# JinPLu/VeloxSeg

Measured on AMD Instinct MI355X. Metric: training patches/s on 128^3 2-mod volumes (fwd+loss+bwd+allreduce+AdamW), higher is better.
Workload: dtype f32

## Files before the change

veloxseg_amd/csrc/expand_mfma.hip:

```cpp
#include "vx_common.h"
#include <type_traits>
#include "../../include/veloxseg_hip.h"

__device__ __forceinline__ int vx_xcd_tile(int bid, int nb) { return (nb & 7) == 0 ? (bid & 7) * (nb >> 3) + (bid >> 3) : bid; }

typedef float vx_f4 __attribute__((ext_vector_type(4)));

__global__ void __launch_bounds__(256) vx_weight_tap_major_k(const float* __restrict__ w, float* __restrict__ wt, int Cout, int Cin, int K3) {
    const long n = (long)Cout * Cin * K3;
    const long e = (long)blockIdx.x * 256 + threadIdx.x;
    if (e >= n) return;
    const int ci = (int)(e % Cin);
    const int co = (int)((e / Cin) % Cout);
    const int t = (int)(e / ((long)Cin * Cout));
    wt[e] = w[((long)co * Cin + ci) * K3 + t];
}

__global__ void __launch_bounds__(256) vx_to_channels_last16_k(const float* __restrict__ x, float* __restrict__ xcl, long V) {
    __shared__ float tile[16][65];
    const int b = blockIdx.y;
    const long v0 = (long)blockIdx.x * 64;
    for (int e = threadIdx.x; e < 16 * 64; e += 256) {
        const int c = e / 64, k = e % 64;
        tile[c][k] = (v0 + k < V) ? x[((long)b * 16 + c) * V + v0 + k] : 0.0f;
// ... 603 lines not shown
    const float* __restrict__ xb = x + (long)b * 16 * V;
    for (int e = threadIdx.x; e < 2 * 648; e += 256) {
        const int hv = e % 648, half = e / 648;
        const int hw = hv % 18, hh = (hv / 18) % 6, hd = hv / 108;
        const int qd = d0 - 1 + hd, qh = h0 - 1 + hh, qw = w0 - 1 + hw;
        const bool ok = (unsigned)qd < (unsigned)D && (unsigned)qh < (unsigned)H && (unsigned)qw < (unsigned)W;
        const float* __restrict__ src = xb + (long)(8 * half) * V + (ok ? ((long)qd * H + qh) * W + qw : 0);
        float v[8];
#pragma unroll
        for (int j = 0; j < 8; ++j) v[j] = src[(long)j * V];
        uint4 pk = make_uint4(0u, 0u, 0u, 0u);
        if (ok) pk = make_uint4(vx_pack_bf16(v[0], v[1]), vx_pack_bf16(v[2], v[3]), vx_pack_bf16(v[4], v[5]), vx_pack_bf16(v[6], v[7]));
        xh[e] = pk;
    }
    __syncthreads();
    const long FH = 4L * H, FW = 4L * W;
    const long fplane = (4L * D) * FH * FW;
    for (int g = 0; g < Cc * 4; ++g) {
        const int c = g >> 2, s1 = g & 3;
        const int co_base = g * 16;
        vx_f4 acc[4];
#pragma unroll
        for (int m = 0; m < 4; ++m) acc[m] = (vx_f4){0.f, 0.f, 0.f, 0.f};
        const uint4* __restrict__ wg = wimg + (long)g * 14 * 64 + lane;
#pragma unroll 2
        for (int p = 0; p < 14; ++p) {
            const int t = 2 * p + (q >> 1);
            const int tt = t < 27 ? t : 26;
            const int tw = tt % 3, th = (tt / 3) % 3, td = tt / 9;
            const uint4 av = wg[p * 64];
            const uint4* __restrict__ xt = xh + (q & 1) * 648 + ((wave + td) * 6 + th) * 18 + r + tw;
            uint4 bv[4];
#pragma unroll
            for (int m = 0; m < 4; ++m) bv[m] = xt[m * 18];
#pragma unroll
            for (int m = 0; m < 4; ++m) acc[m] = __builtin_amdgcn_mfma_f32_16x16x32_bf16(vx_as_bf8(av), vx_as_bf8(bv[m]), acc[m], 0, 0, 0);
        }
        const float4 bb = bias ? *reinterpret_cast<const float4*>(bias + co_base + 4 * q) : make_float4(0.f, 0.f, 0.f, 0.f);
        TY* __restrict__ yb = y + ((long)b * Cc + c) * fplane + ((long)(4 * (d0 + wave) + s1) * FH + q) * FW + 4 * (w0 + r);
#pragma unroll
        for (int m = 0; m < 4; ++m)
            if (w0 + r < W) vx_st4(yb, (long)(4 * (h0 + m)) * FW, make_float4(acc[m][0] + bb.x, acc[m][1] + bb.y, acc[m][2] + bb.z, acc[m][3] + bb.w));
    }
}

extern "C" int vx_expand_fwd_mfma_bf16_h(const float* x, const float* w, const float* bias, float* wt_ws, void* y, int B, int Cc, int D, int H, int W, int y_h16, void* stream) {
    VX_REQUIRE(x && w && wt_ws && y && B > 0 && Cc > 0 && D > 0 && H > 0 && W > 0, "vx_expand_fwd_mfma_bf16: bad args");
    if (D % 4 != 0 || H % 4 != 0 || W % 4 != 0) return 1;
    hipStream_t st = (hipStream_t)stream;
    const int groups = Cc * 4;
    vx_expand_wimg_bf16_k<<<vx_cdiv((long)groups * 14 * 64 * 4, 256), 256, 0, st>>>(w, reinterpret_cast<uint32_t*>(wt_ws), groups, 0);
    const long nblk = (long)B * (D / 4) * (H / 4) * ((W + 15) / 16);
    if (y_h16) vx_expand_fwd_bf16_k<vx_bf16><<<dim3((unsigned)nblk), 256, 0, st>>>(x, reinterpret_cast<const uint4*>(wt_ws), bias, (vx_bf16*)y, B, Cc, D, H, W);
    else vx_expand_fwd_bf16_k<float><<<dim3((unsigned)nblk), 256, 0, st>>>(x, reinterpret_cast<const uint4*>(wt_ws), bias, (float*)y, B, Cc, D, H, W);
    VX_LAUNCH_CHECK("vx_expand_fwd_mfma_bf16");
    return 0;
}
extern "C" int vx_expand_fwd_mfma_bf16(const float* x, const float* w, const float* bias, float* wt_ws, float* y, int B, int Cc, int D, int H, int W, void* stream) {
    return vx_expand_fwd_mfma_bf16_h(x, w, bias, wt_ws, y, B, Cc, D, H, W, 0, stream);
}

template <typename TD>
__global__ void __launch_bounds__(256) vx_expand_bwd_data_bf16_k(const TD* __restrict__ dyf, const uint4* __restrict__ wimg, float* __restrict__ dx,
                                                                 int B, int Cc, int D, int H, int W, int accumulate) {
    extern __shared__ __attribute__((aligned(16))) unsigned short vx_halo_h[];
    const int lane = threadIdx.x & 63;
    const int wave = __builtin_amdgcn_readfirstlane((int)(threadIdx.x >> 6));
    const int r = lane & 15, q = lane >> 4;
    const int nTw = (W + 15) / 16, nTh = H / 4, nTd = D / 4;
    int tile = vx_xcd_tile(blockIdx.x, gridDim.x);
    const int tw_i = tile % nTw; tile /= nTw;
    const int th_i = tile % nTh; tile /= nTh;
    const int td_i = tile % nTd;
    const int b = tile / nTd;
    const int d0 = td_i * 4, h0 = th_i * 4, w0 = tw_i * 16;
    const long V = (long)D * H * W;
    const long FH = 4L * H, FW = 4L * W;
    const long fplane = (4L * D) * FH * FW;
    const TD* __restrict__ dyb = dyf + (long)b * Cc * fplane;
    vx_f4 acc[4];
#pragma unroll
    for (int m = 0; m < 4; ++m) acc[m] = (vx_f4){0.f, 0.f, 0.f, 0.f};
    long goff[11];
    int loff[11];
#pragma unroll
    for (int u = 0; u < 11; ++u) {
        const int e = min((int)threadIdx.x + u * 256, 144 * 18 - 1);
        const int f4 = e % 18, row = e / 18;
        const int s2 = row & 3, hh = (row >> 2) % 6, hd = row / 24;
        const int qd = d0 - 1 + hd, qh = h0 - 1 + hh, qw = w0 - 1 + f4;
        const bool ok = (unsigned)qd < (unsigned)D && (unsigned)qh < (unsigned)H && (unsigned)qw < (unsigned)W;
        goff[u] = ok ? ((long)(4 * qd) * FH + 4 * qh + s2) * FW + 4 * qw : -1;
        loff[u] = ((int)threadIdx.x + u * 256 < 144 * 18) ? (e / 18) * 72 + (e % 18) * 4 : -1;
    }
    for (int c = 0; c < Cc; ++c) {
        for (int s1 = 0; s1 < 4; ++s1) {
            __syncthreads();
            {
                uint2 v[11];
#pragma unroll
                for (int u = 0; u < 11; ++u) {
                    const long o = (long)c * fplane + (goff[u] >= 0 ? goff[u] + (long)s1 * FH * FW : 0);
                    if constexpr (std::is_same<TD, vx_bf16>::value) {
                        const uint2 t_ = *reinterpret_cast<const uint2*>(dyb + o);
                        v[u] = goff[u] >= 0 ? t_ : make_uint2(0u, 0u);
                    } else {
                        const float4 t_ = *reinterpret_cast<const float4*>(dyb + o);
                        v[u] = goff[u] >= 0 ? make_uint2(vx_pack_bf16(t_.x, t_.y), vx_pack_bf16(t_.z, t_.w)) : make_uint2(0u, 0u);
                    }
                }
#pragma unroll
                for (int u = 0; u < 11; ++u)
                    if (loff[u] >= 0) *reinterpret_cast<uint2*>(vx_halo_h + loff[u]) = v[u];
            }
            __syncthreads();
            const uint4* __restrict__ wg = wimg + (long)(c * 4 + s1) * 14 * 64 + lane;
#pragma unroll 2
            for (int p = 0; p < 14; ++p) {
                const int t = 2 * p + (q >> 1);
                const int tt = t < 27 ? t : 26;
                const int tw = tt % 3, th = (tt / 3) % 3, td = tt / 9;
                const uint4 bv = wg[p * 64];
                const int hd = wave - td + 2;
                const int s2 = 2 * (q & 1);
                const unsigned short* __restrict__ ht = vx_halo_h + ((hd * 6 + (2 - th)) * 4 + s2) * 72 + (r - tw + 2) * 4;
                uint4 av[4];
#pragma unroll
                for (int m = 0; m < 4; ++m) {
                    const uint2 lo = *reinterpret_cast<const uint2*>(ht + m * 4 * 72);
                    const uint2 hi = *reinterpret_cast<const uint2*>(ht + m * 4 * 72 + 72);
                    av[m] = make_uint4(lo.x, lo.y, hi.x, hi.y);
                }
#pragma unroll
                for (int m = 0; m < 4; ++m) acc[m] = __builtin_amdgcn_mfma_f32_16x16x32_bf16(vx_as_bf8(av[m]), vx_as_bf8(bv), acc[m], 0, 0, 0);
            }
        }
    }
#pragma unroll
    for (int m = 0; m < 4; ++m) {
        const long pbase = ((long)(d0 + wave) * H + (h0 + m)) * W + w0 + 4 * q;
        float* dst = dx + ((long)b * 16 + r) * V + pbase;
        if (w0 + 4 * q >= W) continue;
        float4 o = make_float4(acc[m][0], acc[m][1], acc[m][2], acc[m][3]);
        if (accumulate) { const float4 old = *reinterpret_cast<float4*>(dst); o.x += old.x; o.y += old.y; o.z += old.z; o.w += old.w; }
        *reinterpret_cast<float4*>(dst) = o;
    }
}

extern "C" int vx_expand_bwd_data_mfma_bf16_h(const void* dy_fine, const float* w, float* wt_ws, float* dx, int B, int Cc, int D, int H, int W,
                                              int accumulate, int dy_h16, void* stream) {
    VX_REQUIRE(dy_fine && w && wt_ws && dx && B > 0 && Cc > 0 && D > 0 && H > 0 && W > 0, "vx_expand_bwd_data_mfma_bf16: bad args");
    if (D % 4 != 0 || H % 4 != 0 || W % 4 != 0) return 1;
    hipStream_t st = (hipStream_t)stream;
    const int groups = Cc * 4;
    vx_expand_wimg_bf16_k<<<vx_cdiv((long)groups * 14 * 64 * 4, 256), 256, 0, st>>>(w, reinterpret_cast<uint32_t*>(wt_ws), groups, 1);
    const long nblk = (long)B * (D / 4) * (H / 4) * ((W + 15) / 16);
    if (dy_h16) vx_expand_bwd_data_bf16_k<vx_bf16><<<dim3((unsigned)nblk), 256, 6 * 6 * 4 * 72 * sizeof(unsigned short), st>>>((const vx_bf16*)dy_fine, reinterpret_cast<const uint4*>(wt_ws), dx, B, Cc, D, H, W, accumulate);
    else vx_expand_bwd_data_bf16_k<float><<<dim3((unsigned)nblk), 256, 6 * 6 * 4 * 72 * sizeof(unsigned short), st>>>((const float*)dy_fine, reinterpret_cast<const uint4*>(wt_ws), dx, B, Cc, D, H, W, accumulate);
    VX_LAUNCH_CHECK("vx_expand_bwd_data_mfma_bf16");
    return 0;
}
extern "C" int vx_expand_bwd_data_mfma_bf16(const float* dy_fine, const float* w, float* wt_ws, float* dx, int B, int Cc, int D, int H, int W,
                                            int accumulate, void* stream) {
    return vx_expand_bwd_data_mfma_bf16_h(dy_fine, w, wt_ws, dx, B, Cc, D, H, W, accumulate, 0, stream);
}


template <int NS>
__device__ __forceinline__ void vx_split8(const float (&v)[8], uint4 (&out)[NS]) {
    float r[8];
#pragma unroll
    for (int j = 0; j < 8; ++j) r[j] = v[j];
#pragma unroll
    for (int s = 0; s < NS; ++s) {
        typedef __bf16 bf2 __attribute__((ext_vector_type(2)));
        uint32_t pk[4];
#pragma unroll
        for (int j2 = 0; j2 < 4; ++j2) {
            const bf2 h = {(__bf16)r[2 * j2], (__bf16)r[2 * j2 + 1]};
            pk[j2] = __builtin_bit_cast(uint32_t, h);
            if (s + 1 < NS) { r[2 * j2] -= (float)h[0]; r[2 * j2 + 1] -= (float)h[1]; }
        }
        out[s] = make_uint4(pk[0], pk[1], pk[2], pk[3]);
    }
}
template <int NS>
__global__ void __launch_bounds__(256) vx_expand_wimg_split_k(const float* __restrict__ w, uint32_t* __restrict__ img, int groups, int backward) {
    const long n = (long)groups * 14 * 64 * 4;
    const long e = (long)blockIdx.x * 256 + threadIdx.x;
    if (e >= n) return;
    const int jp = (int)(e & 3), lane = (int)((e >> 2) & 63);
    const long t = e >> 8;
    const int p = (int)(t % 14), g = (int)(t / 14);
    const int r = lane & 15, q = lane >> 4;
    const int tap = 2 * p + (q >> 1);
    float v[2] = {0.f, 0.f};
    if (tap < 27)
        for (int u = 0; u < 2; ++u) {
            const int j = 2 * jp + u;
            int co, ci;
            if (backward) { co = 16 * g + 4 * (2 * (q & 1) + (j >> 2)) + (j & 3); ci = r; }
            else { co = 16 * g + r; ci = 8 * (q & 1) + j; }
            v[u] = w[((long)co * 16 + ci) * 27 + tap];
        }
#pragma unroll
    for (int s = 0; s < NS; ++s) {
        typedef __bf16 bf2 __attribute__((ext_vector_type(2)));
        const bf2 h = {(__bf16)v[0], (__bf16)v[1]};
        img[(long)s * n + e] = __builtin_bit_cast(uint32_t, h);
        v[0] -= (float)h[0]; v[1] -= (float)h[1];
    }
}
typedef _Float16 vx_h8 __attribute__((ext_vector_type(8)));
__device__ __forceinline__ vx_h8 vx_as_h8(uint4 v) { return __builtin_bit_cast(vx_h8, v); }
__device__ __forceinline__ uint32_t vx_pack_h2(float a, float b) {
    typedef _Float16 h2 __attribute__((ext_vector_type(2)));
    const h2 v = {(_Float16)a, (_Float16)b};
    return __builtin_bit_cast(uint32_t, v);
}
__device__ __forceinline__ float vx_h2_lo(uint32_t p) { typedef _Float16 h2 __attribute__((ext_vector_type(2))); return (float)__builtin_bit_cast(h2, p)[0]; }
__device__ __forceinline__ float vx_h2_hi(uint32_t p) { typedef _Float16 h2 __attribute__((ext_vector_type(2))); return (float)__builtin_bit_cast(h2, p)[1]; }
__device__ __forceinline__ int vx_exp16(float m) {
    if (!(m > 0.0f) || !(m < 3.0e38f)) return 0;
    const int e = 14 - ilogbf(m);
    return e > 100 ? 100 : (e < -100 ? -100 : e);
}
__global__ void __launch_bounds__(256) vx_expand_wmax_k(const float* __restrict__ w, long n, float* __restrict__ out) {
    __shared__ float sm[4];
    float mx = 0.0f;
    const long n4 = n >> 2;
    for (long i = (long)blockIdx.x * 256 + threadIdx.x; i < n4; i += (long)gridDim.x * 256) {
        const float4 t = reinterpret_cast<const float4*>(w)[i];
        mx = fmaxf(mx, fmaxf(fmaxf(fabsf(t.x), fabsf(t.y)), fmaxf(fabsf(t.z), fabsf(t.w))));
    }
    if (blockIdx.x == 0)
        for (long i = 4 * n4 + threadIdx.x; i < n; i += 256) mx = fmaxf(mx, fabsf(w[i]));
    mx = vx_wave_max(mx);
    if ((threadIdx.x & 63) == 0) sm[threadIdx.x >> 6] = mx;
    __syncthreads();
    if (threadIdx.x == 0) out[4 + blockIdx.x] = fmaxf(fmaxf(sm[0], sm[1]), fmaxf(sm[2], sm[3]));
}
__device__ __forceinline__ int vx_expand_wexp(const float* __restrict__ ew) { return vx_exp16(__uint_as_float(reinterpret_cast<const unsigned*>(ew)[1])); }
static inline int vx_expand_wmax_launch(const float* w, long n, float* ew, hipStream_t st) {
    int nb = (int)((n / 4 + 255) / 256);
    if (nb > 64) nb = 64;
    if (nb < 1) nb = 1;
    vx_expand_wmax_k<<<nb, 256, 0, st>>>(w, n, ew);
    return nb;
}
__global__ void __launch_bounds__(256) vx_expand_wimg_f16_k(const float* __restrict__ w, uint32_t* __restrict__ img, const float* __restrict__ ew, int groups, int backward,
                                                            int nparts, float* __restrict__ ew_out) {
    const long n = (long)groups * 14 * 64 * 4;
    const long e = (long)blockIdx.x * 256 + threadIdx.x;
    int wexp;
    if (nparts > 0) {
        float mx = 0.0f;
        for (int i = 0; i < nparts; ++i) mx = fmaxf(mx, ew_out[4 + i]);
        wexp = vx_exp16(mx);
        if (e == 0) { reinterpret_cast<unsigned*>(ew_out)[0] = 0u; reinterpret_cast<unsigned*>(ew_out)[1] = __float_as_uint(mx); }
    } else wexp = vx_expand_wexp(ew);
    if (e >= n) return;
    const float sc = ldexpf(1.0f, wexp);
    const int jp = (int)(e & 3), lane = (int)((e >> 2) & 63);
    const long t = e >> 8;
    const int p = (int)(t % 14), g = (int)(t / 14);
    const int r = lane & 15, q = lane >> 4;
    const int tap = 2 * p + (q >> 1);
    float v[2] = {0.f, 0.f};
    if (tap < 27)
        for (int u = 0; u < 2; ++u) {
            const int j = 2 * jp + u;
            int co, ci;
            if (backward) { co = 16 * g + 4 * (2 * (q & 1) + (j >> 2)) + (j & 3); ci = r; }
            else { co = 16 * g + r; ci = 8 * (q & 1) + j; }
            v[u] = w[((long)co * 16 + ci) * 27 + tap] * sc;
        }
    const uint32_t h0 = vx_pack_h2(v[0], v[1]);
    img[e] = h0;
    img[n + e] = vx_pack_h2(v[0] - vx_h2_lo(h0), v[1] - vx_h2_hi(h0));
}
__device__ __forceinline__ void vx_split8_h(const float (&v)[8], float sc, uint4 (&out)[2]) {
    uint32_t p0[4], p1[4];
#pragma unroll
    for (int j2 = 0; j2 < 4; ++j2) {
        const float a = v[2 * j2] * sc, b = v[2 * j2 + 1] * sc;
        p0[j2] = vx_pack_h2(a, b);
        p1[j2] = vx_pack_h2(a - vx_h2_lo(p0[j2]), b - vx_h2_hi(p0[j2]));
    }
    out[0] = make_uint4(p0[0], p0[1], p0[2], p0[3]);
    out[1] = make_uint4(p1[0], p1[1], p1[2], p1[3]);
}
__device__ __forceinline__ float vx_block_max_256(float m, float* __restrict__ scratch) {
    m = vx_wave_max(m);
    if ((threadIdx.x & 63) == 0) scratch[threadIdx.x >> 6] = m;
    __syncthreads();
    return fmaxf(fmaxf(scratch[0], scratch[1]), fmaxf(scratch[2], scratch[3]));
}

template <int NS> struct VxSplitTerms;
template <> struct VxSplitTerms<1> { static constexpr int N = 1; static constexpr int A[1] = {0}; static constexpr int W[1] = {0}; };
template <> struct VxSplitTerms<2> { static constexpr int N = 3; static constexpr int A[3] = {1, 0, 0}; static constexpr int W[3] = {0, 1, 0}; };
template <> struct VxSplitTerms<3> { static constexpr int N = 6; static constexpr int A[6] = {1, 2, 0, 1, 0, 0}; static constexpr int W[6] = {1, 0, 2, 0, 1, 0}; };

template <int NS, bool F16 = false>
__global__ void __launch_bounds__(256) vx_expand_fwd_split_k(const float* __restrict__ x, const uint4* __restrict__ wimg, const float* __restrict__ bias,
                                                             float* __restrict__ y, int B, int Cc, int D, int H, int W, const float* __restrict__ ew = nullptr) {
    extern __shared__ __attribute__((aligned(16))) uint4 vx_xs[];
    using TT = VxSplitTerms<NS>;
    const int lane = threadIdx.x & 63;
    const int wave = __builtin_amdgcn_readfirstlane((int)(threadIdx.x >> 6));
    const int r = lane & 15, q = lane >> 4;
    const int nTw = (W + 15) / 16, nTh = H / 4, nTd = D / 4;
    int tile = vx_xcd_tile(blockIdx.x, gridDim.x);
    const int tw_i = tile % nTw; tile /= nTw;
    const int th_i = tile % nTh; tile /= nTh;
    const int td_i = tile % nTd;
    const int b = tile / nTd;
    const int d0 = td_i * 4, h0 = th_i * 4, w0 = tw_i * 16;
    const long V = (long)D * H * W;
    const float* __restrict__ xb = x + (long)b * 16 * V;
    float fscale = 1.0f;
    if constexpr (F16) {
        float v[6][8];
        float mx = 0.0f;
#pragma unroll
        for (int i = 0; i < 6; ++i) {
            const int e = (int)threadIdx.x + i * 256;
            const int ec = e < 2 * 648 ? e : 0;
            const int hv = ec % 648, half = ec / 648;
            const int hw = hv % 18, hh = (hv / 18) % 6, hd = hv / 108;
            const int qd = d0 - 1 + hd, qh = h0 - 1 + hh, qw = w0 - 1 + hw;
            const bool ok = e < 2 * 648 && (unsigned)qd < (unsigned)D && (unsigned)qh < (unsigned)H && (unsigned)qw < (unsigned)W;
            const float* __restrict__ src = xb + (long)(8 * half) * V + (ok ? ((long)qd * H + qh) * W + qw : 0);
#pragma unroll
            for (int j = 0; j < 8; ++j) { const float t_ = src[(long)j * V]; v[i][j] = ok ? t_ : 0.0f; mx = fmaxf(mx, fabsf(v[i][j])); }
        }
        float* scratch = reinterpret_cast<float*>(vx_xs + NS * (2 * 648));
        const int ex = vx_exp16(vx_block_max_256(mx, scratch));
        const float sc = ldexpf(1.0f, ex);
        fscale = ldexpf(1.0f, -(ex + vx_expand_wexp(ew)));
#pragma unroll
        for (int i = 0; i < 6; ++i) {
            const int e = (int)threadIdx.x + i * 256;
            if (e < 2 * 648) {
                uint4 pk[2];
                vx_split8_h(v[i], sc, pk);
                vx_xs[e] = pk[0];
                vx_xs[2 * 648 + e] = pk[1];
            }
        }
    } else {
    for (int e = threadIdx.x; e < 2 * 648; e += 256) {
        const int hv = e % 648, half = e / 648;
        const int hw = hv % 18, hh = (hv / 18) % 6, hd = hv / 108;
        const int qd = d0 - 1 + hd, qh = h0 - 1 + hh, qw = w0 - 1 + hw;
        const bool ok = (unsigned)qd < (unsigned)D && (unsigned)qh < (unsigned)H && (unsigned)qw < (unsigned)W;
        const float* __restrict__ src = xb + (long)(8 * half) * V + (ok ? ((long)qd * H + qh) * W + qw : 0);
        float v[8];
#pragma unroll
        for (int j = 0; j < 8; ++j) { const float t_ = src[(long)j * V]; v[j] = ok ? t_ : 0.0f; }
        uint4 pk[NS];
        vx_split8<NS>(v, pk);
#pragma unroll
        for (int s = 0; s < NS; ++s) vx_xs[s * (2 * 648) + e] = pk[s];
    }
    }
    __syncthreads();
    const long FH = 4L * H, FW = 4L * W;
    const long fplane = (4L * D) * FH * FW;
    const long wn = (long)Cc * 4 * 14 * 64;
    for (int g = 0; g < Cc * 4; ++g) {
        const int c = g >> 2, s1 = g & 3;
        const int co_base = g * 16;
        vx_f4 acc[4];
#pragma unroll
        for (int m = 0; m < 4; ++m) acc[m] = (vx_f4){0.f, 0.f, 0.f, 0.f};
        const uint4* __restrict__ wg = wimg + (long)g * 14 * 64 + lane;
#pragma unroll 2
        for (int p = 0; p < 14; ++p) {
            const int t = 2 * p + (q >> 1);
            const int tt = t < 27 ? t : 26;
            const int tw = tt % 3, th = (tt / 3) % 3, td = tt / 9;
            uint4 av[NS], bv[NS][4];
#pragma unroll
            for (int s = 0; s < NS; ++s) {
                av[s] = wg[s * wn + p * 64];
                const uint4* __restrict__ xt = vx_xs + s * (2 * 648) + (q & 1) * 648 + ((wave + td) * 6 + th) * 18 + r + tw;
#pragma unroll
                for (int m = 0; m < 4; ++m) bv[s][m] = xt[m * 18];
            }
#pragma unroll
            for (int k = 0; k < TT::N; ++k)
#pragma unroll
                for (int m = 0; m < 4; ++m) {
                    if constexpr (F16) acc[m] = __builtin_amdgcn_mfma_f32_16x16x32_f16(vx_as_h8(av[TT::W[k]]), vx_as_h8(bv[TT::A[k]][m]), acc[m], 0, 0, 0);
                    else acc[m] = __builtin_amdgcn_mfma_f32_16x16x32_bf16(vx_as_bf8(av[TT::W[k]]), vx_as_bf8(bv[TT::A[k]][m]), acc[m], 0, 0, 0);
                }
        }
        if constexpr (F16) {
#pragma unroll
            for (int m = 0; m < 4; ++m) acc[m] *= fscale;
        }
        const float4 bb = bias ? *reinterpret_cast<const float4*>(bias + co_base + 4 * q) : make_float4(0.f, 0.f, 0.f, 0.f);
        float* __restrict__ yb = y + ((long)b * Cc + c) * fplane + ((long)(4 * (d0 + wave) + s1) * FH + q) * FW + 4 * (w0 + r);
#pragma unroll
        for (int m = 0; m < 4; ++m)
            if (w0 + r < W) *reinterpret_cast<float4*>(yb + (long)(4 * (h0 + m)) * FW) = make_float4(acc[m][0] + bb.x, acc[m][1] + bb.y, acc[m][2] + bb.z, acc[m][3] + bb.w);
    }
}

template <int NS>
__device__ __forceinline__ void vx_split4(const float4 v, uint2 (&out)[NS]) {
    float r[4] = {v.x, v.y, v.z, v.w};
#pragma unroll
    for (int s = 0; s < NS; ++s) {
        typedef __bf16 bf2 __attribute__((ext_vector_type(2)));
        const bf2 h0 = {(__bf16)r[0], (__bf16)r[1]}, h1 = {(__bf16)r[2], (__bf16)r[3]};
        out[s] = make_uint2(__builtin_bit_cast(uint32_t, h0), __builtin_bit_cast(uint32_t, h1));
        if (s + 1 < NS) { r[0] -= (float)h0[0]; r[1] -= (float)h0[1]; r[2] -= (float)h1[0]; r[3] -= (float)h1[1]; }
    }
}
template <int NS, bool F16 = false>
__global__ void __launch_bounds__(256) vx_expand_bwd_data_split_k(const float* __restrict__ dyf, const uint4* __restrict__ wimg, float* __restrict__ dx,
                                                                  int B, int Cc, int D, int H, int W, int accumulate, const float* __restrict__ ew = nullptr) {
    extern __shared__ __attribute__((aligned(16))) uint2 vx_hs[];
    using TT = VxSplitTerms<NS>;
    const int lane = threadIdx.x & 63;
    const int wave = __builtin_amdgcn_readfirstlane((int)(threadIdx.x >> 6));
    const int r = lane & 15, q = lane >> 4;
    const int nTw = (W + 15) / 16, nTh = H / 4, nTd = D / 4;
    int tile = vx_xcd_tile(blockIdx.x, gridDim.x);
    const int tw_i = tile % nTw; tile /= nTw;
    const int th_i = tile % nTh; tile /= nTh;
    const int td_i = tile % nTd;
    const int b = tile / nTd;
    const int d0 = td_i * 4, h0 = th_i * 4, w0 = tw_i * 16;
    const long V = (long)D * H * W;
    const long FH = 4L * H, FW = 4L * W;
    const long fplane = (4L * D) * FH * FW;
    const float* __restrict__ dyb = dyf + (long)b * Cc * fplane;
    const long wn = (long)Cc * 4 * 14 * 64;
    vx_f4 acc[4];
    vx_f4 tot[4];
#pragma unroll
    for (int m = 0; m < 4; ++m) { acc[m] = (vx_f4){0.f, 0.f, 0.f, 0.f}; tot[m] = (vx_f4){0.f, 0.f, 0.f, 0.f}; }
    int soff[11];
    unsigned okm = 0;
#pragma unroll
    for (int u = 0; u < 11; ++u) {
        const int e = min((int)threadIdx.x + u * 256, 144 * 18 - 1);
        const int f4 = e % 18, row = e / 18;
        const int s2 = row & 3, hh = (row >> 2) % 6, hd = row / 24;
        const int qd = d0 - 1 + hd, qh = h0 - 1 + hh, qw = w0 - 1 + f4;
        const bool ok = (unsigned)qd < (unsigned)D && (unsigned)qh < (unsigned)H && (unsigned)qw < (unsigned)W;
        soff[u] = ok ? (int)(((long)(4 * qd) * FH + 4 * qh + s2) * FW + 4 * qw) : 0;
        okm |= (ok ? 1u : 0u) << u;
    }
    const long s1stride = FH * FW;
    for (int c = 0; c < Cc; ++c) {
        for (int s1 = 0; s1 < 4; ++s1) {
            __syncthreads();
            float gscale = 1.0f;
            {
                float4 v[11];
                const float* __restrict__ cb_ = dyb + (long)c * fplane + (long)s1 * s1stride;
#pragma unroll
                for (int u = 0; u < 11; ++u) {
                    const bool ok = (okm >> u) & 1u;
                    const float4 t_ = *reinterpret_cast<const float4*>(ok ? cb_ + soff[u] : dyb);
                    v[u] = ok ? t_ : make_float4(0.f, 0.f, 0.f, 0.f);
                }
                if constexpr (F16) {
                    float mx = 0.0f;
#pragma unroll
                    for (int u = 0; u < 11; ++u) mx = fmaxf(mx, fmaxf(fmaxf(fabsf(v[u].x), fabsf(v[u].y)), fmaxf(fabsf(v[u].z), fabsf(v[u].w))));
                    const int ex = vx_exp16(vx_block_max_256(mx, reinterpret_cast<float*>(vx_hs + NS * (144 * 18))));
                    const float sc = ldexpf(1.0f, ex);
                    gscale = ldexpf(1.0f, -(ex + vx_expand_wexp(ew)));
#pragma unroll
                    for (int u = 0; u < 11; ++u) {
                        const int e = (int)threadIdx.x + u * 256;
                        if (e < 144 * 18) {
                            const float a0 = v[u].x * sc, a1 = v[u].y * sc, a2 = v[u].z * sc, a3 = v[u].w * sc;
                            const uint32_t l0 = vx_pack_h2(a0, a1), h0 = vx_pack_h2(a2, a3);
                            vx_hs[e] = make_uint2(l0, h0);
                            vx_hs[144 * 18 + e] = make_uint2(vx_pack_h2(a0 - vx_h2_lo(l0), a1 - vx_h2_hi(l0)), vx_pack_h2(a2 - vx_h2_lo(h0), a3 - vx_h2_hi(h0)));
                        }
                    }
                } else {
#pragma unroll
                for (int u = 0; u < 11; ++u) {
                    const int e = (int)threadIdx.x + u * 256;
                    if (e < 144 * 18) {
                        uint2 pc[NS];
                        vx_split4<NS>(v[u], pc);
#pragma unroll
                        for (int s = 0; s < NS; ++s) vx_hs[s * (144 * 18) + e] = pc[s];
                    }
                }
                }
            }
            __syncthreads();
            const uint4* __restrict__ wg = wimg + (long)(c * 4 + s1) * 14 * 64 + lane;
#pragma unroll 2
            for (int p = 0; p < 14; ++p) {
                const int t = 2 * p + (q >> 1);
                const int tt = t < 27 ? t : 26;
                const int tw = tt % 3, th = (tt / 3) % 3, td = tt / 9;
                uint4 bv[NS];
#pragma unroll
                for (int s = 0; s < NS; ++s) bv[s] = wg[s * wn + p * 64];
                const int hd = wave - td + 2;
                const int s2 = 2 * (q & 1);
                const uint2* __restrict__ ht = vx_hs + ((hd * 6 + (2 - th)) * 4 + s2) * 18 + (r - tw + 2);
                uint4 av[4][NS];
#pragma unroll
                for (int s = 0; s < NS; ++s)
#pragma unroll
                    for (int m = 0; m < 4; ++m) {
                        const uint2 lo = ht[s * (144 * 18) + m * 4 * 18], hi = ht[s * (144 * 18) + m * 4 * 18 + 18];
                        av[m][s] = make_uint4(lo.x, lo.y, hi.x, hi.y);
                    }
#pragma unroll
                for (int k = 0; k < TT::N; ++k)
#pragma unroll
                    for (int m = 0; m < 4; ++m) {
                        if constexpr (F16) acc[m] = __builtin_amdgcn_mfma_f32_16x16x32_f16(vx_as_h8(av[m][TT::A[k]]), vx_as_h8(bv[TT::W[k]]), acc[m], 0, 0, 0);
                        else acc[m] = __builtin_amdgcn_mfma_f32_16x16x32_bf16(vx_as_bf8(av[m][TT::A[k]]), vx_as_bf8(bv[TT::W[k]]), acc[m], 0, 0, 0);
                    }
            }
            if constexpr (F16) {
#pragma unroll
                for (int m = 0; m < 4; ++m) { tot[m] += acc[m] * gscale; acc[m] = (vx_f4){0.f, 0.f, 0.f, 0.f}; }
            }
        }
    }
    if constexpr (F16) {
#pragma unroll
        for (int m = 0; m < 4; ++m) acc[m] = tot[m];
    }
#pragma unroll
    for (int m = 0; m < 4; ++m) {
        const long pbase = ((long)(d0 + wave) * H + (h0 + m)) * W + w0 + 4 * q;
        float* dst = dx + ((long)b * 16 + r) * V + pbase;
        if (w0 + 4 * q >= W) continue;
        float4 o = make_float4(acc[m][0], acc[m][1], acc[m][2], acc[m][3]);
        if (accumulate) { const float4 old = *reinterpret_cast<float4*>(dst); o.x += old.x; o.y += old.y; o.z += old.z; o.w += old.w; }
        *reinterpret_cast<float4*>(dst) = o;
    }
}

extern "C" int vx_expand_split_ws_floats(int Cc, int ns) { return (Cc <= 0 || !(ns == 2 || ns == 3 || ns == 22)) ? -1 : Cc * 4 * 14 * 64 * 4 * (ns == 22 ? 2 : ns) + (ns == 22 ? 4 + 64 : 0); }

extern "C" int vx_expand_fwd_mfma_split(const float* x, const float* w, const float* bias, float* wt_ws, float* y, int B, int Cc, int D, int H, int W, int ns, void* stream) {
    VX_REQUIRE(x && w && wt_ws && y && B > 0 && Cc > 0 && D > 0 && H > 0 && W > 0 && (ns == 2 || ns == 3 || ns == 22), "vx_expand_fwd_mfma_split: bad args");
    if (D % 4 != 0 || H % 4 != 0 || W % 4 != 0) return 1;
    hipStream_t st = (hipStream_t)stream;
    const int groups = Cc * 4;
    const long nblk = (long)B * (D / 4) * (H / 4) * ((W + 15) / 16);
    const size_t shm = (size_t)(ns == 22 ? 2 : ns) * 2 * 648 * sizeof(uint4) + (ns == 22 ? 32 : 0);
    if (ns == 22) {
        float* ew = wt_ws + (long)groups * 14 * 64 * 4 * 2;
        const int nparts = vx_expand_wmax_launch(w, (long)groups * 16 * 16 * 27, ew, st);
        vx_expand_wimg_f16_k<<<vx_cdiv((long)groups * 14 * 64 * 4, 256), 256, 0, st>>>(w, reinterpret_cast<uint32_t*>(wt_ws), ew, groups, 0, nparts, ew);
        vx_expand_fwd_split_k<2, true><<<dim3((unsigned)nblk), 256, shm, st>>>(x, reinterpret_cast<const uint4*>(wt_ws), bias, y, B, Cc, D, H, W, ew);
    } else if (ns == 2) {
        vx_expand_wimg_split_k<2><<<vx_cdiv((long)groups * 14 * 64 * 4, 256), 256, 0, st>>>(w, reinterpret_cast<uint32_t*>(wt_ws), groups, 0);
        vx_expand_fwd_split_k<2><<<dim3((unsigned)nblk), 256, shm, st>>>(x, reinterpret_cast<const uint4*>(wt_ws), bias, y, B, Cc, D, H, W);
    } else {
        vx_expand_wimg_split_k<3><<<vx_cdiv((long)groups * 14 * 64 * 4, 256), 256, 0, st>>>(w, reinterpret_cast<uint32_t*>(wt_ws), groups, 0);
        vx_expand_fwd_split_k<3><<<dim3((unsigned)nblk), 256, shm, st>>>(x, reinterpret_cast<const uint4*>(wt_ws), bias, y, B, Cc, D, H, W);
    }
    VX_LAUNCH_CHECK("vx_expand_fwd_mfma_split");
    return 0;
}
extern "C" int vx_expand_prep_split22(const float* w, float* wt_fwd, float* wt_bwd, int Cc, void* stream) {
    VX_REQUIRE(w && wt_fwd && wt_bwd && Cc > 0, "vx_expand_prep_split22: bad args");
    hipStream_t st = (hipStream_t)stream;
    const int groups = Cc * 4;
    float* ew = wt_fwd + (long)groups * 14 * 64 * 4 * 2;
    const int nparts = vx_expand_wmax_launch(w, (long)groups * 16 * 16 * 27, ew, st);
    const unsigned nb = (unsigned)vx_cdiv((long)groups * 14 * 64 * 4, 256);
    vx_expand_wimg_f16_k<<<nb, 256, 0, st>>>(w, reinterpret_cast<uint32_t*>(wt_fwd), ew, groups, 0, nparts, ew);
    vx_expand_wimg_f16_k<<<nb, 256, 0, st>>>(w, reinterpret_cast<uint32_t*>(wt_bwd), ew, groups, 1, 0, nullptr);
    VX_LAUNCH_CHECK("vx_expand_prep_split22");
    return 0;
}
extern "C" int vx_expand_fwd_mfma_split_prepared(const float* x, const float* bias, const float* wt_fwd, float* y, int B, int Cc, int D, int H, int W, void* stream) {
    VX_REQUIRE(x && wt_fwd && y && B > 0 && Cc > 0 && D > 0 && H > 0 && W > 0, "vx_expand_fwd_mfma_split_prepared: bad args");
    if (D % 4 != 0 || H % 4 != 0 || W % 4 != 0) return 1;
    const int groups = Cc * 4;
    const long nblk = (long)B * (D / 4) * (H / 4) * ((W + 15) / 16);
    const size_t shm = (size_t)2 * 2 * 648 * sizeof(uint4) + 32;
    vx_expand_fwd_split_k<2, true><<<dim3((unsigned)nblk), 256, shm, (hipStream_t)stream>>>(x, reinterpret_cast<const uint4*>(wt_fwd), bias, y, B, Cc, D, H, W, wt_fwd + (long)groups * 14 * 64 * 4 * 2);
    VX_LAUNCH_CHECK("vx_expand_fwd_mfma_split_prepared");
    return 0;
}
extern "C" int vx_expand_bwd_data_mfma_split_prepared(const float* dy_fine, const float* wt_bwd, const float* ew_fwd, float* dx, int B, int Cc, int D, int H, int W, int accumulate,
                                                      void* stream) {
    VX_REQUIRE(dy_fine && wt_bwd && ew_fwd && dx && B > 0 && Cc > 0 && D > 0 && H > 0 && W > 0, "vx_expand_bwd_data_mfma_split_prepared: bad args");
    if (D % 4 != 0 || H % 4 != 0 || W % 4 != 0) return 1;
    const long nblk = (long)B * (D / 4) * (H / 4) * ((W + 15) / 16);
    const size_t shm = (size_t)2 * 144 * 18 * sizeof(uint2) + 32;
    vx_expand_bwd_data_split_k<2, true><<<dim3((unsigned)nblk), 256, shm, (hipStream_t)stream>>>(dy_fine, reinterpret_cast<const uint4*>(wt_bwd), dx, B, Cc, D, H, W, accumulate, ew_fwd);
    VX_LAUNCH_CHECK("vx_expand_bwd_data_mfma_split_prepared");
    return 0;
}
extern "C" int vx_expand_bwd_data_mfma_split_ew(const float* dy_fine, const float* w, float* wt_ws, float* dx, int B, int Cc, int D, int H, int W, int accumulate, int ns,
                                                const float* ew_fwd, void* stream);
extern "C" int vx_expand_bwd_data_mfma_split(const float* dy_fine, const float* w, float* wt_ws, float* dx, int B, int Cc, int D, int H, int W, int accumulate, int ns,
                                             void* stream) {
    return vx_expand_bwd_data_mfma_split_ew(dy_fine, w, wt_ws, dx, B, Cc, D, H, W, accumulate, ns, nullptr, stream);
}
extern "C" int vx_expand_split_ew_offset(int Cc) { return Cc * 4 * 14 * 64 * 4 * 2; }
extern "C" int vx_expand_bwd_data_mfma_split_ew(const float* dy_fine, const float* w, float* wt_ws, float* dx, int B, int Cc, int D, int H, int W, int accumulate, int ns,
                                                const float* ew_fwd, void* stream) {
    VX_REQUIRE(dy_fine && w && wt_ws && dx && B > 0 && Cc > 0 && D > 0 && H > 0 && W > 0 && (ns == 2 || ns == 3 || ns == 22), "vx_expand_bwd_data_mfma_split: bad args");
    if (D % 4 != 0 || H % 4 != 0 || W % 4 != 0) return 1;
    hipStream_t st = (hipStream_t)stream;
    const int groups = Cc * 4;
    const long nblk = (long)B * (D / 4) * (H / 4) * ((W + 15) / 16);
    const size_t shm = (size_t)(ns == 22 ? 2 : ns) * 144 * 18 * sizeof(uint2) + (ns == 22 ? 32 : 0);
    if (ns == 22) {
        float* ew_own = wt_ws + (long)groups * 14 * 64 * 4 * 2;
        const int nparts = ew_fwd == nullptr ? vx_expand_wmax_launch(w, (long)groups * 16 * 16 * 27, ew_own, st) : 0;
        const float* ew = ew_fwd ? ew_fwd : ew_own;
        vx_expand_wimg_f16_k<<<vx_cdiv((long)groups * 14 * 64 * 4, 256), 256, 0, st>>>(w, reinterpret_cast<uint32_t*>(wt_ws), ew, groups, 1, nparts, ew_own);
        vx_expand_bwd_data_split_k<2, true><<<dim3((unsigned)nblk), 256, shm, st>>>(dy_fine, reinterpret_cast<const uint4*>(wt_ws), dx, B, Cc, D, H, W, accumulate, ew);
    } else if (ns == 2) {
        vx_expand_wimg_split_k<2><<<vx_cdiv((long)groups * 14 * 64 * 4, 256), 256, 0, st>>>(w, reinterpret_cast<uint32_t*>(wt_ws), groups, 1);
        vx_expand_bwd_data_split_k<2><<<dim3((unsigned)nblk), 256, shm, st>>>(dy_fine, reinterpret_cast<const uint4*>(wt_ws), dx, B, Cc, D, H, W, accumulate);
    } else {
        vx_expand_wimg_split_k<3><<<vx_cdiv((long)groups * 14 * 64 * 4, 256), 256, 0, st>>>(w, reinterpret_cast<uint32_t*>(wt_ws), groups, 1);
        vx_expand_bwd_data_split_k<3><<<dim3((unsigned)nblk), 256, shm, st>>>(dy_fine, reinterpret_cast<const uint4*>(wt_ws), dx, B, Cc, D, H, W, accumulate);
    }
    VX_LAUNCH_CHECK("vx_expand_bwd_data_mfma_split");
    return 0;
}

#define VX_WS_PITCH 20
template <int NS, typename TD = float>
__global__ void __launch_bounds__(256, 3) vx_expand_wgrad_split_k(const float* __restrict__ x, const TD* __restrict__ dyf, float* __restrict__ part, float* __restrict__ db,
                                                                   int B, int Cc, int D, int H, int W, int HL, int nHs, int nWc, int nUnits) {
    extern __shared__ __attribute__((aligned(16))) uint32_t vx_wx[];
    using TT = VxSplitTerms<NS>;
    const int lane = threadIdx.x & 63;
    const int wave = __builtin_amdgcn_readfirstlane((int)(threadIdx.x >> 6));
    const int r = lane & 15, q = lane >> 4;
    const int xcd = blockIdx.x & 7, m_ = blockIdx.x >> 3;
    const int pd = m_ % 3, unit = (m_ / 3) * 8 + xcd;
    if (unit >= nUnits) return;
    const int c = unit % Cc;
    int strip = unit / Cc;
    const int strip_id = strip;
    const int wc = strip % nWc; strip /= nWc;
    const int hs = strip % nHs; strip /= nHs;
    const int d = strip % D;
    const int b = strip / D;
    const int dq = d - 1 + pd;
    if ((unsigned)dq >= (unsigned)D) return;
    const int h_lo = hs * HL, h_hi = (h_lo + HL < H) ? h_lo + HL : H, wc0 = wc * 32;
    const long V = (long)D * H * W;
    const float* __restrict__ xb = x + (long)b * 16 * V + (long)dq * H * W;
    float4 pf = make_float4(0.f, 0.f, 0.f, 0.f);
    const int st_ci = (threadIdx.x >> 3) & 15, st_seg = threadIdx.x & 7;
    auto fetch = [&](int hq) {
        if (threadIdx.x < 128) {
            const int w = wc0 + 4 * st_seg;
            pf = ((unsigned)hq < (unsigned)H && w < W) ? *reinterpret_cast<const float4*>(xb + (long)st_ci * V + (long)hq * W + w) : make_float4(0.f, 0.f, 0.f, 0.f);
        }
    };
    auto stash = [&](int hq) {
        if (threadIdx.x < 128) {
            const int slot = hq & 3;
            uint2 pk[NS];
            vx_split4<NS>(pf, pk);
#pragma unroll
            for (int s = 0; s < NS; ++s) *reinterpret_cast<uint2*>(vx_wx + (((s * 4 + slot) * 16 + st_ci) * VX_WS_PITCH + 2 * st_seg)) = pk[s];
        }
    };
    const int s1 = wave, s2 = r >> 2, s3 = r & 3;
    const long FH = 4L * H, FW = 4L * W;
    const TD* __restrict__ dyb = dyf + (((long)b * Cc + c) * (4L * D) + 4 * d + s1) * FH * FW + (long)s2 * FW + 4L * (wc0 + 8 * q) + s3;
    float dv[10];
    auto fetch_dy = [&](int h) {
        const TD* __restrict__ p = dyb + 4L * h * FW;
#pragma unroll
        for (int j = 0; j < 10; ++j) {
            const int w = wc0 + 8 * q + j - 1;
            dv[j] = (h < h_hi && (unsigned)w < (unsigned)W) ? vx_ld1(p, 4L * (j - 1)) : 0.0f;
        }
    };
    vx_f4 acc[9];
#pragma unroll
    for (int t = 0; t < 9; ++t) acc[t] = (vx_f4){0.f, 0.f, 0.f, 0.f};
    float bsum = 0.0f;
    for (int hq = h_lo - 1; hq <= h_lo + 1; ++hq) { fetch(hq); stash(hq); }
    fetch_dy(h_lo);
    __syncthreads();
    for (int h = h_lo; h < h_hi; ++h) {
        uint4 a[NS][3];
        {
            float rr[10];
#pragma unroll
            for (int j = 0; j < 10; ++j) rr[j] = dv[j];
#pragma unroll
            for (int j = 1; j < 9; ++j) bsum += dv[j];
#pragma unroll
            for (int s = 0; s < NS; ++s) {
                typedef __bf16 bf2 __attribute__((ext_vector_type(2)));
                uint32_t p[4];
#pragma unroll
                for (int j2 = 0; j2 < 4; ++j2) {
                    const bf2 hh = {(__bf16)rr[1 + 2 * j2], (__bf16)rr[2 + 2 * j2]};
                    p[j2] = __builtin_bit_cast(uint32_t, hh);
                    if (s + 1 < NS) { rr[1 + 2 * j2] -= (float)hh[0]; rr[2 + 2 * j2] -= (float)hh[1]; }
                }
                const bf2 he = {(__bf16)rr[9], (__bf16)rr[0]};
                if (s + 1 < NS) { rr[9] -= (float)he[0]; rr[0] -= (float)he[1]; }
                const uint32_t ends = __builtin_bit_cast(uint32_t, he);
                const uint32_t s01 = __builtin_amdgcn_alignbit(p[1], p[0], 16), s12 = __builtin_amdgcn_alignbit(p[2], p[1], 16), s23 = __builtin_amdgcn_alignbit(p[3], p[2], 16);
                a[s][1] = make_uint4(p[0], p[1], p[2], p[3]);
                a[s][2] = make_uint4(__builtin_amdgcn_alignbit(p[0], ends, 16), s01, s12, s23);
                a[s][0] = make_uint4(s01, s12, s23, __builtin_amdgcn_alignbit(ends, p[3], 16));
            }
        }
        const bool more = h + 1 < h_hi;
        if (more) { fetch(h + 2); fetch_dy(h + 1); }
#pragma unroll
        for (int ph = 0; ph < 3; ++ph) {
            const int slot = (h - 1 + ph) & 3;
            uint4 bv[NS];
#pragma unroll
            for (int s = 0; s < NS; ++s) bv[s] = *reinterpret_cast<const uint4*>(vx_wx + (((s * 4 + slot) * 16 + r) * VX_WS_PITCH + 4 * q));
#pragma unroll
            for (int tw = 0; tw < 3; ++tw)
#pragma unroll
                for (int k = 0; k < TT::N; ++k)
                    acc[ph * 3 + tw] = __builtin_amdgcn_mfma_f32_16x16x32_bf16(vx_as_bf8(a[TT::W[k]][tw]), vx_as_bf8(bv[TT::A[k]]), acc[ph * 3 + tw], 0, 0, 0);
        }
        if (more) stash(h + 2);
        __syncthreads();
    }
    float* __restrict__ red = reinterpret_cast<float*>(vx_wx);
#pragma unroll
    for (int t = 0; t < 9; ++t)
#pragma unroll
        for (int reg = 0; reg < 4; ++reg) red[wave * 2304 + ((4 * q + reg) * 16 + r) * 9 + t] = acc[t][reg];
    __syncthreads();
    float4* __restrict__ prow = reinterpret_cast<float4*>(part + (((long)strip_id * Cc + c) * 3 + pd) * 9216);
    for (int e = threadIdx.x; e < 2304; e += 256) prow[e] = reinterpret_cast<const float4*>(red)[e];
    if (db != nullptr && pd == 1) {
        bsum += __shfl_xor(bsum, 16, 64);
        bsum += __shfl_xor(bsum, 32, 64);
        if (q == 0) atomicAdd(db + (c * 4 + s1) * 16 + r, bsum);
    }
}
__global__ void __launch_bounds__(256) vx_expand_wgrad_fold_k(const float* __restrict__ part, float* __restrict__ dw, int Cc, int D, int nStrips, int perD) {
    __shared__ float4 sm[16][16];
    const int i = threadIdx.x & 15, k = threadIdx.x >> 4;
    const int o4 = blockIdx.x * 16 + i;
    const int total4 = Cc * 3 * 2304;
    float4 s = make_float4(0.f, 0.f, 0.f, 0.f);
    int c = 0, pd = 0, e4 = 0;
    if (o4 < total4) {
        e4 = o4 % 2304;
        pd = (o4 / 2304) % 3;
        c = o4 / (3 * 2304);
        const float4* __restrict__ p4 = reinterpret_cast<const float4*>(part) + ((long)c * 3 + pd) * 2304 + e4;
        const long stride4 = (long)Cc * 3 * 2304;
#pragma unroll 4
        for (int st = k; st < nStrips; st += 16) {
            const int d = (st / perD) % D;
            if ((unsigned)(d - 1 + pd) < (unsigned)D) {
                const float4 v = p4[(long)st * stride4];
                s.x += v.x; s.y += v.y; s.z += v.z; s.w += v.w;
            }
        }
    }
    sm[k][i] = s;
    __syncthreads();
    if (k == 0 && o4 < total4) {
        float4 v = sm[0][i];
#pragma unroll
        for (int kk = 1; kk < 16; ++kk) { const float4 u = sm[kk][i]; v.x += u.x; v.y += u.y; v.z += u.z; v.w += u.w; }
        const float vv[4] = {v.x, v.y, v.z, v.w};
#pragma unroll
        for (int u = 0; u < 4; ++u) {
            const int e = 4 * e4 + u;
            const int wv = e / 2304, rem = e - wv * 2304, cc = rem / 9, t = rem - cc * 9;
            dw[((long)c * 4 + wv) * 6912 + cc * 27 + 9 * pd + t] += vv[u];
        }
    }
}

static void vx_wgs_plan(int B, int Cc, int D, int H, int W, int& HL, int& nHs, int& nWc) {
    nWc = (W + 31) / 32;
    const long base = (long)B * D * nWc * Cc * 3;
    constexpr long target = 384;
    int want = (int)((target + base - 1) / base);
    if (want < 1) want = 1;
    HL = (H + want - 1) / want;
    if (HL < 8) HL = H < 8 ? H : 8;
    nHs = (H + HL - 1) / HL;
}
extern "C" int vx_expand_wgrad_split_ws_floats(int B, int Cc, int D, int H, int W) {
    if (B <= 0 || Cc <= 0 || D <= 0 || H <= 0 || W <= 0) return -1;
    int HL, nHs, nWc;
    vx_wgs_plan(B, Cc, D, H, W, HL, nHs, nWc);
    const long n = (long)B * D * nHs * nWc * Cc * 3 * 9216;
    return n > 0x7fffffffL ? -1 : (int)n;
}
extern "C" int vx_expand_wgrad_mfma_split_h(const float* x, const void* dy_fine_, float* dw, float* db, float* part_ws, long ws_floats, int B, int Cc, int D, int H, int W,
                                            int ns, int dy_h16, void* stream) {
    const float* dy_fine = (const float*)dy_fine_;
    VX_REQUIRE(x && dy_fine && dw && part_ws && B > 0 && Cc > 0 && D > 0 && H > 0 && W > 0 && ns >= 1 && ns <= 3, "vx_expand_wgrad_mfma_split: bad args");
    VX_REQUIRE(!dy_h16 || ns == 1, "vx_expand_wgrad_mfma_split: a 16-bit gradient needs plain bf16 operands (ns = 1)");
    if (W % 4 != 0) return 1;
    int HL, nHs, nWc;
    vx_wgs_plan(B, Cc, D, H, W, HL, nHs, nWc);
    const long nStrips = (long)B * D * nHs * nWc;
    VX_REQUIRE(ws_floats >= nStrips * Cc * 3 * 9216, "vx_expand_wgrad_mfma_split: workspace too small");
    const size_t shm = (size_t)ns * 4 * 16 * VX_WS_PITCH * sizeof(uint32_t);
    const size_t need = 4 * 2304 * sizeof(float);
    const size_t lds = shm > need ? shm : need;
    const int nUnits = (int)(nStrips * Cc);
    dim3 grid((unsigned)(((nUnits + 7) / 8) * 8 * 3));
    if (ns == 1 && dy_h16) vx_expand_wgrad_split_k<1, vx_bf16><<<grid, 256, lds, (hipStream_t)stream>>>(x, (const vx_bf16*)dy_fine_, part_ws, db, B, Cc, D, H, W, HL, nHs, nWc, nUnits);
    else if (ns == 1) vx_expand_wgrad_split_k<1><<<grid, 256, lds, (hipStream_t)stream>>>(x, dy_fine, part_ws, db, B, Cc, D, H, W, HL, nHs, nWc, nUnits);
    else if (ns == 2) vx_expand_wgrad_split_k<2><<<grid, 256, lds, (hipStream_t)stream>>>(x, dy_fine, part_ws, db, B, Cc, D, H, W, HL, nHs, nWc, nUnits);
    else vx_expand_wgrad_split_k<3><<<grid, 256, lds, (hipStream_t)stream>>>(x, dy_fine, part_ws, db, B, Cc, D, H, W, HL, nHs, nWc, nUnits);
    vx_expand_wgrad_fold_k<<<vx_cdiv((long)Cc * 3 * 2304, 16), 256, 0, (hipStream_t)stream>>>(part_ws, dw, Cc, D, (int)nStrips, nHs * nWc);
    VX_LAUNCH_CHECK("vx_expand_wgrad_mfma_split");
    return 0;
}
extern "C" int vx_expand_wgrad_mfma_split(const float* x, const float* dy_fine, float* dw, float* db, float* part_ws, long ws_floats, int B, int Cc, int D, int H, int W,
                                          int ns, void* stream) {
    return vx_expand_wgrad_mfma_split_h(x, dy_fine, dw, db, part_ws, ws_floats, B, Cc, D, H, W, ns, 0, stream);
}
```

Baseline: 1072.

## Prefetch expand weights through register ring and double-buffer wgrad row loads

In the forward and backward-data expand kernels, the per-tap weight loads from global memory are replaced by a 4-deep register ring. Each load is issued several taps ahead, and scheduling barriers keep the compiler from collapsing the pipeline. The backward-data kernel also prefetches the next channel group's dy tile before the current group's MFMA loop. The wgrad kernel double-buffers input and dy row fetches two rows ahead, using clamped addresses instead of predicated loads, which lets all threads stage data. Together these hide global load latency behind MFMA work, at the cost of more VGPRs, which may lower occupancy.

```diff
diff --git a/veloxseg_amd/csrc/expand_mfma.hip b/veloxseg_amd/csrc/expand_mfma.hip
--- a/veloxseg_amd/csrc/expand_mfma.hip
+++ b/veloxseg_amd/csrc/expand_mfma.hip
@@ -929,6 +929,7 @@
 template <> struct VxSplitTerms<2> { static constexpr int N = 3; static constexpr int A[3] = {1, 0, 0}; static constexpr int W[3] = {0, 1, 0}; };
 template <> struct VxSplitTerms<3> { static constexpr int N = 6; static constexpr int A[6] = {1, 2, 0, 1, 0, 0}; static constexpr int W[6] = {1, 0, 2, 0, 1, 0}; };
 
+#define VX_EW_RING 4
 template <int NS, bool F16 = false>
 __global__ void __launch_bounds__(256) vx_expand_fwd_split_k(const float* __restrict__ x, const uint4* __restrict__ wimg, const float* __restrict__ bias,
                                                              float* __restrict__ y, int B, int Cc, int D, int H, int W, const float* __restrict__ ew = nullptr) {
@@ -996,25 +997,44 @@
     const long FH = 4L * H, FW = 4L * W;
     const long fplane = (4L * D) * FH * FW;
     const long wn = (long)Cc * 4 * 14 * 64;
-    for (int g = 0; g < Cc * 4; ++g) {
+    const int nimg = Cc * 4 * 14;
+    const uint4* __restrict__ wl = wimg + lane;
+    uint4 wr[VX_EW_RING][NS];
+#pragma unroll
+    for (int i = 0; i < VX_EW_RING; ++i) {
+#pragma unroll
+        for (int s = 0; s < NS; ++s) wr[i][s] = wl[s * wn + i * 64];
+        __builtin_amdgcn_sched_barrier(0);
+    }
+    for (int g2 = 0; g2 < Cc * 2; ++g2) {
+#pragma unroll
+    for (int gg = 0; gg < 2; ++gg) {
+        const int g = 2 * g2 + gg;
         const int c = g >> 2, s1 = g & 3;
         const int co_base = g * 16;
         vx_f4 acc[4];
 #pragma unroll
         for (int m = 0; m < 4; ++m) acc[m] = (vx_f4){0.f, 0.f, 0.f, 0.f};
-        const uint4* __restrict__ wg = wimg + (long)g * 14 * 64 + lane;
-#pragma unroll 2
+        const float4 bb = bias ? *reinterpret_cast<const float4*>(bias + co_base + 4 * q) : make_float4(0.f, 0.f, 0.f, 0.f);
+#pragma unroll
         for (int p = 0; p < 14; ++p) {
             const int t = 2 * p + (q >> 1);
             const int tt = t < 27 ? t : 26;
             const int tw = tt % 3, th = (tt / 3) % 3, td = tt / 9;
+            const int slot = (gg * 14 + p) % VX_EW_RING;
             uint4 av[NS], bv[NS][4];
 #pragma unroll
             for (int s = 0; s < NS; ++s) {
-                av[s] = wg[s * wn + p * 64];
+                av[s] = wr[slot][s];
                 const uint4* __restrict__ xt = vx_xs + s * (2 * 648) + (q & 1) * 648 + ((wave + td) * 6 + th) * 18 + r + tw;
 #pragma unroll
                 for (int m = 0; m < 4; ++m) bv[s][m] = xt[m * 18];
+            }
+            {
+                const int nx = g * 14 + p + VX_EW_RING;
+                const uint4* __restrict__ wnx = wl + (long)(nx < nimg ? nx : nimg - 1) * 64;
+#pragma unroll
+                for (int s = 0; s < NS; ++s) wr[slot][s] = wnx[s * wn];
             }
 #pragma unroll
             for (int k = 0; k < TT::N; ++k)
@@ -1023,16 +1043,17 @@
                     if constexpr (F16) acc[m] = __builtin_amdgcn_mfma_f32_16x16x32_f16(vx_as_h8(av[TT::W[k]]), vx_as_h8(bv[TT::A[k]][m]), acc[m], 0, 0, 0);
                     else acc[m] = __builtin_amdgcn_mfma_f32_16x16x32_bf16(vx_as_bf8(av[TT::W[k]]), vx_as_bf8(bv[TT::A[k]][m]), acc[m], 0, 0, 0);
                 }
+            __builtin_amdgcn_sched_barrier(0);
         }
         if constexpr (F16) {
 #pragma unroll
             for (int m = 0; m < 4; ++m) acc[m] *= fscale;
         }
-        const float4 bb = bias ? *reinterpret_cast<const float4*>(bias + co_base + 4 * q) : make_float4(0.f, 0.f, 0.f, 0.f);
         float* __restrict__ yb = y + ((long)b * Cc + c) * fplane + ((long)(4 * (d0 + wave) + s1) * FH + q) * FW + 4 * (w0 + r);
 #pragma unroll
         for (int m = 0; m < 4; ++m)
             if (w0 + r < W) *reinterpret_cast<float4*>(yb + (long)(4 * (h0 + m)) * FW) = make_float4(acc[m][0] + bb.x, acc[m][1] + bb.y, acc[m][2] + bb.z, acc[m][3] + bb.w);
+    }
     }
 }
 
@@ -1084,19 +1105,33 @@
         okm |= (ok ? 1u : 0u) << u;
     }
     const long s1stride = FH * FW;
-    for (int c = 0; c < Cc; ++c) {
-        for (int s1 = 0; s1 < 4; ++s1) {
+    float4 v[11];
+    auto fetch_group = [&](int g) {
+        const float* __restrict__ cb_ = dyb + (long)(g >> 2) * fplane + (long)(g & 3) * s1stride;
+#pragma unroll
+        for (int u = 0; u < 11; ++u) {
+            const bool ok = (okm >> u) & 1u;
+            const float4 t_ = *reinterpret_cast<const float4*>(cb_ + soff[u]);
+            v[u] = ok ? t_ : make_float4(0.f, 0.f, 0.f, 0.f);
+        }
+    };
+    const int nimg = Cc * 4 * 14;
+    const uint4* __restrict__ wl = wimg + lane;
+    uint4 wr[VX_EW_RING][NS];
+    fetch_group(0);
+#pragma unroll
+    for (int i = 0; i < VX_EW_RING; ++i) {
+#pragma unroll
+        for (int s = 0; s < NS; ++s) wr[i][s] = wl[s * wn + i * 64];
+        __builtin_amdgcn_sched_barrier(0);
+    }
+    for (int g2 = 0; g2 < Cc * 2; ++g2) {
+#pragma unroll
+        for (int gg = 0; gg < 2; ++gg) {
+            const int g = 2 * g2 + gg;
             __syncthreads();
             float gscale = 1.0f;
             {
-                float4 v[11];
-                const float* __restrict__ cb_ = dyb + (long)c * fplane + (long)s1 * s1stride;
-#pragma unroll
-                for (int u = 0; u < 11; ++u) {
-                    const bool ok = (okm >> u) & 1u;
-                    const float4 t_ = *reinterpret_cast<const float4*>(ok ? cb_ + soff[u] : dyb);
-                    v[u] = ok ? t_ : make_float4(0.f, 0.f, 0.f, 0.f);
-                }
                 if constexpr (F16) {
                     float mx = 0.0f;
 #pragma unroll
@@ -1128,15 +1163,22 @@
                 }
             }
             __syncthreads();
-            const uint4* __restrict__ wg = wimg + (long)(c * 4 + s1) * 14 * 64 + lane;
-#pragma unroll 2
+            fetch_group(g + 1 < Cc * 4 ? g + 1 : g);
+#pragma unroll
             for (int p = 0; p < 14; ++p) {
                 const int t = 2 * p + (q >> 1);
                 const int tt = t < 27 ? t : 26;
                 const int tw = tt % 3, th = (tt / 3) % 3, td = tt / 9;
+                const int slot = (gg * 14 + p) % VX_EW_RING;
                 uint4 bv[NS];
 #pragma unroll
-                for (int s = 0; s < NS; ++s) bv[s] = wg[s * wn + p * 64];
+                for (int s = 0; s < NS; ++s) bv[s] = wr[slot][s];
+                {
+                    const int nx = g * 14 + p + VX_EW_RING;
+                    const uint4* __restrict__ wnx = wl + (long)(nx < nimg ? nx : nimg - 1) * 64;
+#pragma unroll
+                    for (int s = 0; s < NS; ++s) wr[slot][s] = wnx[s * wn];
+                }
                 const int hd = wave - td + 2;
                 const int s2 = 2 * (q & 1);
                 const uint2* __restrict__ ht = vx_hs + ((hd * 6 + (2 - th)) * 4 + s2) * 18 + (r - tw + 2);
@@ -1155,6 +1197,7 @@
                         if constexpr (F16) acc[m] = __builtin_amdgcn_mfma_f32_16x16x32_f16(vx_as_h8(av[m][TT::A[k]]), vx_as_h8(bv[TT::W[k]]), acc[m], 0, 0, 0);
                         else acc[m] = __builtin_amdgcn_mfma_f32_16x16x32_bf16(vx_as_bf8(av[m][TT::A[k]]), vx_as_bf8(bv[TT::W[k]]), acc[m], 0, 0, 0);
                     }
+                __builtin_amdgcn_sched_barrier(0);
             }
             if constexpr (F16) {
 #pragma unroll
@@ -1289,50 +1332,55 @@
     const int h_lo = hs * HL, h_hi = (h_lo + HL < H) ? h_lo + HL : H, wc0 = wc * 32;
     const long V = (long)D * H * W;
     const float* __restrict__ xb = x + (long)b * 16 * V + (long)dq * H * W;
-    float4 pf = make_float4(0.f, 0.f, 0.f, 0.f);
     const int st_ci = (threadIdx.x >> 3) & 15, st_seg = threadIdx.x & 7;
-    auto fetch = [&](int hq) {
-        if (threadIdx.x < 128) {
-            const int w = wc0 + 4 * st_seg;
-            pf = ((unsigned)hq < (unsigned)H && w < W) ? *reinterpret_cast<const float4*>(xb + (long)st_ci * V + (long)hq * W + w) : make_float4(0.f, 0.f, 0.f, 0.f);
-        }
+    const int st_w = wc0 + 4 * st_seg;
+    const float* __restrict__ xrow = xb + (long)st_ci * V + (st_w < W ? st_w : W - 4);
+    auto fetch = [&](int hq, float4& pf) {
+        const int hc = hq < 0 ? 0 : (hq < H ? hq : H - 1);
+        pf = *reinterpret_cast<const float4*>(xrow + (long)hc * W);
     };
-    auto stash = [&](int hq) {
-        if (threadIdx.x < 128) {
-            const int slot = hq & 3;
-            uint2 pk[NS];
-            vx_split4<NS>(pf, pk);
-#pragma unroll
-            for (int s = 0; s < NS; ++s) *reinterpret_cast<uint2*>(vx_wx + (((s * 4 + slot) * 16 + st_ci) * VX_WS_PITCH + 2 * st_seg)) = pk[s];
-        }
+    auto stash = [&](int hq, const float4& pf) {
+        const int slot = hq & 3;
+        const bool ok = (unsigned)hq < (unsigned)H && st_w < W;
+        uint2 pk[NS];
+        vx_split4<NS>(ok ? pf : make_float4(0.f, 0.f, 0.f, 0.f), pk);
+#pragma unroll
+        for (int s = 0; s < NS; ++s) *reinterpret_cast<uint2*>(vx_wx + (((s * 4 + slot) * 16 + st_ci) * VX_WS_PITCH + 2 * st_seg)) = pk[s];
     };
     const int s1 = wave, s2 = r >> 2, s3 = r & 3;
     const long FH = 4L * H, FW = 4L * W;
-    const TD* __restrict__ dyb = dyf + (((long)b * Cc + c) * (4L * D) + 4 * d + s1) * FH * FW + (long)s2 * FW + 4L * (wc0 + 8 * q) + s3;
-    float dv[10];
-    auto fetch_dy = [&](int h) {
-        const TD* __restrict__ p = dyb + 4L * h * FW;
-#pragma unroll
-        for (int j = 0; j < 10; ++j) {
-            const int w = wc0 + 8 * q + j - 1;
-            dv[j] = (h < h_hi && (unsigned)w < (unsigned)W) ? vx_ld1(p, 4L * (j - 1)) : 0.0f;
-        }
+    const TD* __restrict__ dyb = dyf + (((long)b * Cc + c) * (4L * D) + 4 * d + s1) * FH * FW + (long)s2 * FW + s3;
+    int dyo[10];
+#pragma unroll
+    for (int j = 0; j < 10; ++j) { const int w = wc0 + 8 * q + j - 1; dyo[j] = 4 * (w < 0 ? 0 : (w < W ? w : W - 1)); }
+    auto fetch_dy = [&](int h, float (&dv)[10]) {
+        const TD* __restrict__ p = dyb + 4L * (h < h_hi ? h : h_hi - 1) * FW;
+#pragma unroll
+        for (int j = 0; j < 10; ++j) dv[j] = vx_ld1(p, (long)dyo[j]);
     };
     vx_f4 acc[9];
 #pragma unroll
     for (int t = 0; t < 9; ++t) acc[t] = (vx_f4){0.f, 0.f, 0.f, 0.f};
     float bsum = 0.0f;
-    for (int hq = h_lo - 1; hq <= h_lo + 1; ++hq) { fetch(hq); stash(hq); }
-    fetch_dy(h_lo);
+    float dv[2][10];
+    float4 pf[2];
+    {
+        float4 p0, p1, p2;
+        fetch(h_lo - 1, p0); fetch(h_lo, p1); fetch(h_lo + 1, p2);
+        fetch(h_lo + 2, pf[0]);
+        fetch_dy(h_lo, dv[0]);
+        fetch_dy(h_lo + 1, dv[1]);
+        stash(h_lo - 1, p0); stash(h_lo, p1); stash(h_lo + 1, p2);
+    }
     __syncthreads();
-    for (int h = h_lo; h < h_hi; ++h) {
+    auto row = [&](const int h, float (&dvc)[10], float4& pf_near, float4& pf_far) {
         uint4 a[NS][3];
         {
             float rr[10];
 #pragma unroll
-            for (int j = 0; j < 10; ++j) rr[j] = dv[j];
-#pragma unroll
-            for (int j = 1; j < 9; ++j) bsum += dv[j];
+            for (int j = 0; j < 10; ++j) rr[j] = (unsigned)(wc0 + 8 * q + j - 1) < (unsigned)W ? dvc[j] : 0.0f;
+#pragma unroll
+            for (int j = 1; j < 9; ++j) bsum += rr[j];
 #pragma unroll
             for (int s = 0; s < NS; ++s) {
                 typedef __bf16 bf2 __attribute__((ext_vector_type(2)));
@@ -1352,8 +1400,8 @@
                 a[s][0] = make_uint4(s01, s12, s23, __builtin_amdgcn_alignbit(ends, p[3], 16));
             }
         }
-        const bool more = h + 1 < h_hi;
-        if (more) { fetch(h + 2); fetch_dy(h + 1); }
+        fetch(h + 3, pf_far);
+        fetch_dy(h + 2, dvc);
 #pragma unroll
         for (int ph = 0; ph < 3; ++ph) {
             const int slot = (h - 1 + ph) & 3;
@@ -1366,9 +1414,15 @@
                 for (int k = 0; k < TT::N; ++k)
                     acc[ph * 3 + tw] = __builtin_amdgcn_mfma_f32_16x16x32_bf16(vx_as_bf8(a[TT::W[k]][tw]), vx_as_bf8(bv[TT::A[k]]), acc[ph * 3 + tw], 0, 0, 0);
         }
-        if (more) stash(h + 2);
+        stash(h + 2, pf_near);
         __syncthreads();
-    }
+    };
+    int h = h_lo;
+    for (; h + 1 < h_hi; h += 2) {
+        row(h, dv[0], pf[0], pf[1]);
+        row(h + 1, dv[1], pf[1], pf[0]);
+    }
+    if (h < h_hi) row(h, dv[0], pf[0], pf[1]);
     float* __restrict__ red = reinterpret_cast<float*>(vx_wx);
 #pragma unroll
     for (int t = 0; t < 9; ++t)
```

Measured after the change: 1064. About the same (-0.8%).
